# TheCacophonyProject/classifier-pipeline

Measured on AMD Instinct MI355X. Metric: CPTV frames/s end-to-end (track+classify) at 160x120, higher is better.
Workload: dtype u16/i32 track stage (f32 normalise, f64 gates); f32 crop/tile; f32 CNN (stride-1 3x3 convs of stages 2-4 (+ the stride-2 one): two fp16 planes per operand rounded to nearest (11 + 11 significand bits), power-of-two range scaling, 3 fp16 MFMAs per K step, device-side rerun in the exact split if an ac

## Files before the change

### classifier-pipeline_amd/csrc/cpx_api.cpp

```cpp
#include <hip/hip_runtime.h>

#include <algorithm>
#include <cmath>
#include <cstdio>
#include <cstdlib>
#include <cstring>
#include <new>
#include <string>
#include <vector>

#include "cpx_internal.h"
#include "cpx_schedule_core.h"

static_assert(sizeof(cpx_component) == 32, "cpx_component layout is part of the ABI");
static_assert(sizeof(cpx_frame_info) == 80, "cpx_frame_info layout is part of the ABI");
static_assert(sizeof(cpx_frame_meta) == 24, "cpx_frame_meta layout is part of the ABI");
static_assert(sizeof(cpx_config) == 48, "cpx_config layout is part of the ABI");
static_assert(sizeof(cpx_region_ref) == 24 && sizeof(cpx_track_limits) == 32 && sizeof(cpx_crop_req) == 32,
              "classification request layouts are part of the ABI");
static_assert(sizeof(cpx_filter_params) == 72 && sizeof(cpx_track_summary) == 120,
              "end-of-clip layouts are part of the ABI");
static_assert(sizeof(cpx_region) == 56, "cpx_region layout is part of the ABI");
static_assert(sizeof(cpx_track_record) == 32, "cpx_track_record layout is part of the ABI");
static_assert(sizeof(cpx_track_params) == 120, "cpx_track_params layout is part of the ABI");
// ... 79 lines not shown
    return CPX_ERR_HIP;
  }
  h->wtab_len = 65536;
  h->wtab_host.resize(h->wtab_len);
  std::vector<double>& wt = h->wtab_host;
  double w = 0.0;
  for (int k = 0; k < h->wtab_len; ++k) {
    wt[k] = w;
    w = w + cfg->weight_add;
  }
  if (cfg->denoise) {
    if (!cpx::nlm_supported(W, H)) {
      cpx_destroy(h);
      return CPX_ERR_UNSUPPORTED;
    }
    const int fixed_point_mult = (int)(2147483647LL / (21 * 21 * 255));
    std::vector<int> lut(64, 0);
    for (int a2 = 0; a2 < 64; ++a2) {
      const double wv = std::exp(-((double)a2 * (64.0 / 49.0)) / 9.0);
      const double wr = std::nearbyint((double)fixed_point_mult * wv);
      lut[a2] = (wr < 0.001 * fixed_point_mult) ? 0 : (int)wr;
    }
    if (lut[63] != 0 || h->nlm_lut_dev.grow(h, 64 * sizeof(int), "NLM weight table allocation") ||
        hipMemcpy(h->nlm_lut_dev.p, lut.data(), 64 * sizeof(int), hipMemcpyHostToDevice) != hipSuccess) {
      cpx_destroy(h);
      return CPX_ERR_HIP;
    }
  }
  std::vector<uint32_t> thr(h->wtab_len);
  for (int k = 0; k < h->wtab_len; ++k) {
    const double wk = wt[k], m = std::nearbyint(wk);
    const bool exact = (wk == m), near = !exact && std::fabs(wk - m) < 1e-6;
    double hi = near ? m + 1.0 : std::floor(wk) + 1.0;
    if (!(hi >= 0.0)) hi = 0.0;
    if (hi > 536870912.0) hi = 536870912.0;
    thr[k] = 2u * (uint32_t)hi - (near ? 1u : 0u);
  }
  if (h->wthr_dev.grow(h, thr.size() * sizeof(uint32_t), "threshold table allocation") ||
      hipMemcpy(h->wthr_dev.p, thr.data(), thr.size() * sizeof(uint32_t), hipMemcpyHostToDevice) != hipSuccess) {
    cpx_destroy(h);
    return CPX_ERR_HIP;
  }
  if (h->wtab_dev.grow(h, wt.size() * sizeof(double), "weight table allocation") ||
      hipMemcpy(h->wtab_dev.p, wt.data(), wt.size() * sizeof(double), hipMemcpyHostToDevice) != hipSuccess ||
      cpx::frame_kernel_attr_setup() != 0) {
    cpx_destroy(h);
    return CPX_ERR_HIP;
  }
  if (const char* env = std::getenv("CPX_TRACK_PACKED_STATE")) h->packed_state_ok = std::atoi(env) != 0;
  if (const char* env = std::getenv("CPX_CNN_FUSE_CONV1")) h->fuse_conv1 = std::atoi(env) != 0;
  if (const char* env = std::getenv("CPX_TRACK_PER_STEP")) h->track_per_step = std::atoi(env) != 0;
  if (const char* env = std::getenv("CPX_CNN_FUSE_SHORTCUT")) h->fuse_shortcut = std::atoi(env) != 0;
  if (const char* env = std::getenv("CPX_CNN_SHORTCUT_FP16")) h->shortcut_fp16 = std::atoi(env) != 0;
  if (const char* env = std::getenv("CPX_CNN_BLOCK_FUSION")) h->block_fusion = std::min(std::max(std::atoi(env), 0), 2);
  if (const char* env = std::getenv("CPX_CNN_MATH")) {
    if (!std::strcmp(env, "f32")) h->cnn_math = CPX_CNN_MATH_F32;
    else if (!std::strcmp(env, "bf16x3")) h->cnn_math = CPX_CNN_MATH_BF16X3;
    else if (!std::strcmp(env, "bf16x2")) h->cnn_math = CPX_CNN_MATH_BF16X2;
    else if (!std::strcmp(env, "fp16x2")) h->cnn_math = CPX_CNN_MATH_FP16X2;
  }
  *out = h;
  return CPX_OK;
}

static void release_buffers(cpx_handle* h, bool all) {
  for (DeviceBuffer* b : {&h->ws, &h->ws_assoc, &h->bf3_scratch, &h->cnn_arena, &h->graph_arena, &h->ir_scratch}) b->release();
  if (!all) return;
  for (DeviceBuffer* b : {&h->sched, &h->wtab_dev, &h->wthr_dev, &h->nlm_lut_dev, &h->cnn_ovf, &h->ir_bitmap}) b->release();
}

void cpx_destroy(cpx_handle* h) {
  if (!h) return;
  hipSetDevice(h->device);
  if (h->stream) hipStreamSynchronize(h->stream);
  for (cpx_cnn* c : h->cnns) cnn_free(c);
  h->cnns.clear();
  for (cpx_mog2* m : h->mog2s) mog2_free(m);
  h->mog2s.clear();
  for (cpx_graph* g : h->graphs) graph_free(g);
  h->graphs.clear();
  release_buffers(h, true);
  for (auto& e : h->conv_events) {
    hipEventDestroy(e.e0);
    hipEventDestroy(e.e1);
  }
  if (h->stream2) {
    hipStreamSynchronize(h->stream2);
    hipStreamDestroy(h->stream2);
  }
  if (h->ev_median) hipEventDestroy(h->ev_median);
  if (h->ev0) hipEventDestroy(h->ev0);
  if (h->ev1) hipEventDestroy(h->ev1);
  if (h->stream) hipStreamDestroy(h->stream);
  delete h;
}

const char* cpx_last_error(const cpx_handle* h) { return h ? h->err.c_str() : "null handle"; }

void* cpx_stream(cpx_handle* h) { return h ? (void*)h->stream : nullptr; }

static int join_medians(cpx_handle* h) {
  if (h->medians_pending) {
    h->medians_pending = false;
    CPX_HIP(h, hipStreamWaitEvent(h->stream, h->ev_median, 0));
  }
  return CPX_OK;
// ... 711 lines not shown
```

### classifier-pipeline_amd/csrc/cpx_api_cnn.cpp

```cpp
#include <hip/hip_runtime.h>

#include <algorithm>
#include <cmath>
#include <cstdio>
#include <cstdlib>
#include <new>
#include <utility>
#include <vector>

#include "cpx_internal.h"

static_assert(sizeof(cpx_wrresnet_block) == 56 && sizeof(cpx_wrresnet_params) == 1560,
              "cpx_wrresnet_params layout is part of the ABI");

struct cpx_cnn {
  cpx_handle* h = nullptr;
  cpx_wrresnet_params p{};
  std::vector<std::pair<const float*, void*>> split;
  float act_scale[3][CPX_WRRESNET_MAX_BLOCKS][2];
  float res_bound[3] = {0.0f, 0.0f, 0.0f};
  float sc_xscale[3] = {0.0f, 0.0f, 0.0f};
  void* sc_img[3] = {nullptr, nullptr, nullptr};
  double sc_wmax[3] = {-1.0, -1.0, -1.0};
  cpx_cnn() {
// ... 65 lines not shown
    a.sc_H = fuse->H; a.sc_W = fuse->W; a.sc_cin = fuse->cin; a.sc_stride = fuse->stride;
    a.sc_planes = fuse->planes; a.sc_xscale = fuse->xscale;
  }
  return a;
}

class ConvTimer {
 public:
  ConvTimer(cpx_handle* h, bool on) : h_(h) {
    if (!on) return;
    ok_ = hipEventCreate(&ev_.e0) == hipSuccess && hipEventCreate(&ev_.e1) == hipSuccess &&
          hipEventRecord(ev_.e0, h->stream) == hipSuccess;
  }
  ~ConvTimer() {
    if (ev_.e0) hipEventDestroy(ev_.e0);
    if (ev_.e1) hipEventDestroy(ev_.e1);
  }
  ConvTimer(const ConvTimer&) = delete;
  ConvTimer& operator=(const ConvTimer&) = delete;
  bool ok() const { return ok_; }
  int commit(int key, double flops) {
    if (!ev_.e0) return CPX_OK;
    CPX_HIP(h_, hipEventRecord(ev_.e1, h_->stream));
    ev_.key = key;
    ev_.flops = flops;
    h_->conv_events.push_back(ev_);
    ev_ = {};
    return CPX_OK;
  }

 private:
  cpx_handle* h_;
  cpx_handle::ConvEv ev_{};
  bool ok_ = true;
};

enum class ConvRoute {
  Float32,
  Split,
  Fp16Pair,
  RerunOnly,
};

static int conv_run(cpx_handle* h, const cpx_conv_desc* d, const void* split_weights, const conv_fuse* fuse = nullptr,
                    const conv_half* hf = nullptr) {
  if (!h) return CPX_ERR_INVALID;
  if (!d || !d->in_dev || !d->out_dev || !d->weights_dev) return fail(h, CPX_ERR_INVALID, "cpx_conv2d: null argument");
  if (d->N < 1 || d->H < 1 || d->W < 1 || d->groups < 1 || d->Cin % d->groups || d->Cout % d->groups ||
      d->ksize < 1 || d->stride < 1 || (d->in_scale_dev == nullptr) != (d->in_shift_dev == nullptr))
    return fail(h, CPX_ERR_INVALID, "cpx_conv2d: bad descriptor");
  CPX_ENTER(h);
  if (!d->pad_same && (d->H < d->ksize || d->W < d->ksize)) return fail(h, CPX_ERR_INVALID, "cpx_conv2d: input smaller than kernel");
  cpx::ConvArgs a = conv_describe(*d, fuse);
  const bool split = split_math(h) && cpx::conv_bf3_supported(a);
  if (fuse && (!split || a.out_scale || a.residual))
    return fail(h, CPX_ERR_INVALID, "conv_run: shortcut fusion needs the split-operand kernel, no output scale, no residual");
  if (split) a.planes = h->cnn_math == CPX_CNN_MATH_BF16X2 ? 2 : 3;
  const conv_half bare;
  const conv_half& k = hf ? *hf : bare;
  const bool fp16 = split && h->cnn_math == CPX_CNN_MATH_FP16X2;
  const bool aliased = a.out == a.residual || a.out == a.in;
  const bool half = fp16 && cpx::conv_bf3_two_planes(a) && !aliased;
  const bool planes_out = fp16 && k.out_planes;
  const ConvRoute route = k.rerun_only ? ConvRoute::RerunOnly
                          : !split ? ConvRoute::Float32
                          : (half || planes_out) ? ConvRoute::Fp16Pair
                                                 : ConvRoute::Split;
  ConvTimer timer(h, h->conv_timing && route != ConvRoute::RerunOnly);
  if (!timer.ok()) return fail(h, CPX_ERR_HIP, "cpx_conv2d: event creation failed");
  int* word = nullptr;
  if (route == ConvRoute::Fp16Pair || route == ConvRoute::RerunOnly) {
    if (int rc = ensure_ovf_word(h)) return rc;
    if (!k.keep_flag) CPX_HIP(h, hipMemsetAsync(h->cnn_ovf.p, 0, sizeof(int), h->stream));
    word = h->cnn_ovf.as<int>() + k.word;
  }
  if (split && !split_weights) {
    if (int rc = h->bf3_scratch.grow(h, cpx::conv_bf3_weight_bytes(a), "cpx_conv2d: weight scratch allocation failed"))
      return rc;
    cpx::launch_split_weights(a, h->bf3_scratch.p, h->stream);
    split_weights = h->bf3_scratch.p;
  }
  int rc = 0;
  if (route == ConvRoute::Fp16Pair) {
    cpx::ConvArgs first = a;
    if (half) {
      first.planes = 2;
      first.half = 1;
      first.act_scale = k.act_scale;
      first.act_unscale = 1.0f / first.act_scale;
      first.in_planes = k.in_planes;
    }
    first.ovf = word;
    if (planes_out) {
      first.out_planes = 1;
      first.out_act_scale = k.out_act_scale;
    }
    rc = cpx::launch_conv_bf3(first, split_weights, h->stream);
  }
  a.guard = word;
  if (split) {
    if (rc == 0) rc = cpx::launch_conv_bf3(a, split_weights, h->stream);
    if (rc == -3) {
      if (fuse) return fail(h, CPX_ERR_UNSUPPORTED, "conv_run: batch too large for the fused-shortcut kernel (split the call)");
      rc = cpx::launch_conv(a, h->stream);
    }
  } else {
    rc = cpx::launch_conv(a, h->stream);
// ... 573 lines not shown
```

### classifier-pipeline_amd/csrc/cpx_cnn_rw.hip

```cpp
#include <hip/hip_runtime.h>

#include <algorithm>
#include <type_traits>

#include "cpx_kernels.h"

namespace cpx {

namespace {

typedef unsigned u32x4 __attribute__((ext_vector_type(4)));
typedef float f32x4 __attribute__((ext_vector_type(4)));
typedef _Float16 f16x2 __attribute__((ext_vector_type(2)));
typedef _Float16 f16x8 __attribute__((ext_vector_type(8)));

template <typename T>
__device__ __forceinline__ const T* at_off(const T* base, unsigned bytes) {
  return reinterpret_cast<const T*>(reinterpret_cast<const char*>(base) + bytes);
}
template <typename T>
__device__ __forceinline__ T* at_off(T* base, unsigned bytes) {
  return reinterpret_cast<T*>(reinterpret_cast<char*>(base) + bytes);
}
__device__ __forceinline__ unsigned pix_off(int y, int x, int W, int C) {
  return __umul24(__umul24((unsigned)y, (unsigned)W) + (unsigned)x, (unsigned)C);
}
__device__ __forceinline__ float relu_bits(float x) { return __int_as_float(max(__float_as_int(x), 0)); }
__device__ __forceinline__ void split_h(float a, float b, unsigned& hi, unsigned& lo) {
  f16x2 v = {(_Float16)a, (_Float16)b};
  hi = __builtin_bit_cast(unsigned, v);
  asm("v_fma_mixlo_f16 %0, %1, 1.0, -%2 op_sel:[0,0,0] op_sel_hi:[0,0,1]" : "=v"(lo) : "v"(a), "v"(hi));
  asm("v_fma_mixhi_f16 %0, %1, 1.0, -%2 op_sel:[0,0,1] op_sel_hi:[0,0,1]" : "+v"(lo) : "v"(b), "v"(hi));
}
__device__ __forceinline__ f32x4 mfma_h(u32x4 w, u32x4 x, f32x4 c) {
  return __builtin_amdgcn_mfma_f32_16x16x32_f16(__builtin_bit_cast(f16x8, w), __builtin_bit_cast(f16x8, x), c, 0, 0, 0);
}

struct RwTiles {
  unsigned long long m_tx, m_ty;
  int tiles_x, tiles_y, total;
};
template <int I, int N, typename F>
__device__ __forceinline__ void static_for(F&& f) {
  if constexpr (I < N) {
    f(std::integral_constant<int, I>{});
    static_for<I + 1, N>(f);
  }
}
__device__ __forceinline__ int div_magic(int n, unsigned long long m) { return (int)(((unsigned long long)n * m) >> 42); }

constexpr int RW_TW = 16;
constexpr int RW_CT = 256;
constexpr int RW_PPI = RW_CT / 8;
constexpr int RW_WC = 64;

template <int S, int NCH, int ROWS>
struct RwGeo {
  static constexpr int PW = 15 * S + 3, PH = (ROWS - 1) * S + 3, NPX = PH * PW;
  static constexpr int NP = (NPX * 8 + RW_CT - 1) / RW_CT;
  static constexpr int NPXP = (NP * RW_PPI + 3) / 4 * 4 + 2;
  static constexpr int BUF = 2 * 2 * NPXP * 2;
  static constexpr int STEPS = 3 * PH;
  static constexpr int CING = 32 * NCH;
  static constexpr size_t LDS = (size_t)2 * BUF * 16 + (size_t)(2 * CING + 3 * RW_WC) * sizeof(float);
};
constexpr int SC_NPXP = 258;
constexpr int SC_ITEMS = 16 * RW_TW * 8 / RW_CT;
constexpr size_t SC_LDS = (size_t)2 * 2 * SC_NPXP * 2 * 16;

template <int S, int NCH, int ROWS, bool BN, bool RES, bool SC = false>
__global__ __launch_bounds__(RW_CT) __attribute__((amdgpu_waves_per_eu(1, 1))) void conv_rw_kernel(ConvArgs a, const uint4* __restrict__ wimg, RwTiles td) {
  using G = RwGeo<S, NCH, ROWS>;
  constexpr int PW = G::PW, NPX = G::NPX, NP = G::NP, NPXP = G::NPXP, BUF = G::BUF, STEPS = G::STEPS, CING = G::CING, PH = G::PH;
  static_assert(!SC || (S == 1 && NCH == 2 && ROWS == 16 && !RES), "the fp16 shortcut is built into the stride-1 form's two-chunk stream");
  if (*a.ovf != 0) return;
  extern __shared__ __attribute__((aligned(16))) uint4 lds4[];
  uint4* s_buf = lds4;
  float* s_bn = reinterpret_cast<float*>(lds4 + 2 * BUF);
  float* s_par = s_bn + 2 * CING;
  uint4* s_sc = reinterpret_cast<uint4*>(s_par + 3 * RW_WC);
  const int tid = threadIdx.x, lane = tid & 63, wave = tid >> 6, i16 = lane & 15, q = lane >> 4;
  const int ct = wave;
  const int cout_g = a.Cout / a.groups, nhalf = cout_g / RW_WC;
  const int g = blockIdx.y / nhalf, half = blockIdx.y - g * nhalf;
  constexpr bool has_bn = BN;

  u32x4 Wr[NCH][9][2];
  {
    const u32x4* wg = reinterpret_cast<const u32x4*>(wimg) + (size_t)g * NCH * 3 * 24 * cout_g + (q * cout_g + half * RW_WC + ct * 16 + i16);
#pragma unroll
    for (int c = 0; c < NCH; ++c)
#pragma unroll
      for (int ky = 0; ky < 3; ++ky)
#pragma unroll
        for (int kx = 0; kx < 3; ++kx)
#pragma unroll
          for (int p = 0; p < 2; ++p) Wr[c][ky * 3 + kx][p] = wg[(size_t)((c * 3 + ky) * 24 + (p * 3 + kx) * 4) * cout_g];
  }
  u32x4 Wsc[2];
  if constexpr (SC) {
    const u32x4* ws = reinterpret_cast<const u32x4*>(a.sc_planes) + (size_t)g * 8 * cout_g + (q * cout_g + half * RW_WC + ct * 16 + i16);
    Wsc[0] = ws[0];
    Wsc[1] = ws[(size_t)4 * cout_g];
  }
  if (tid < CING) {
    const int ci = g * CING + tid;
    s_bn[tid] = has_bn ? a.in_scale[ci] * a.act_scale : a.act_scale;
    s_bn[CING + tid] = has_bn ? a.in_shift[ci] * a.act_scale : 0.0f;
  }
  if (tid < RW_WC) {
    const int ch = g * cout_g + half * RW_WC + tid;
    float os = a.w_unscale[ch] * a.act_unscale;
    if (a.out_scale) os *= a.out_scale[ch];
    float ob = a.out_shift ? a.out_shift[ch] : 0.0f;
    if (a.sc_in && a.sc_bias) ob += a.sc_bias[ch];
    s_par[tid] = os;
    s_par[RW_WC + tid] = ob;
    s_par[2 * RW_WC + tid] = a.w_scale[ch] * a.act_scale;
  }

  const int per_xcd = (td.total + 7) >> 3;
  auto tile_of = [&](int t) { return (t & 7) * per_xcd + (t >> 3); };
  auto decode = [&](int tile, int& n_, int& oy_, int& ox_) {
    int qd = div_magic(tile, td.m_tx);
    ox_ = (tile - qd * td.tiles_x) * RW_TW;
    tile = qd;
    qd = div_magic(tile, td.m_ty);
// ... 53 lines not shown
    const int iy = oy_ * S - a.pad_top + (ipos[i] >> 8), ix = ox_ * S - a.pad_left + (ipos[i] & 0xFF);
    const bool inside = (unsigned)iy < (unsigned)a.H && (unsigned)ix < (unsigned)a.W;
#pragma unroll
    for (int j = 0; j < 4; ++j) pre_p[i][j] = __float_as_uint(inside ? v[j] : 0.0f);
  };
  auto store_item = [&](const int i, const int bsel) __attribute__((always_inline)) {
    unsigned h0, h1, l0, l1;
    split_h(__uint_as_float(pre_p[i][0]), __uint_as_float(pre_p[i][1]), h0, l0);
    split_h(__uint_as_float(pre_p[i][2]), __uint_as_float(pre_p[i][3]), h1, l1);
    if (has_bn) hmax = pk_max_u16(pk_max_u16(hmax, h0), h1);
    else hmax = pk_max_u16(pk_max_u16(hmax, h0 & 0x7FFF7FFFu), h1 & 0x7FFF7FFFu);
    unsigned char* sp = reinterpret_cast<unsigned char*>(s_buf) + st_base;
    *reinterpret_cast<uint2*>(sp + (bsel * BUF * 16 + i * (RW_PPI * 32))) = make_uint2(h0, h1);
    *reinterpret_cast<uint2*>(sp + (bsel * BUF * 16 + 2 * NPXP * 32 + i * (RW_PPI * 32))) = make_uint2(l0, l1);
  };

  u32x4 pre_s[SC ? SC_ITEMS : 1];
  u32x4 xsh[2], xsl[2];
  const unsigned sc_st_base = (unsigned)((((q8 >> 2) * SC_NPXP + (tid >> 3)) * 4 + (q8 & 3)) * 8);
  const int sc_a_base = ((q >> 1) * SC_NPXP + i16) * 2 + (q & 1);
  auto issue_sc = [&](const int i, const int n_, const int oy_, const int ox_) __attribute__((always_inline)) {
    if constexpr (SC) {
      const float* sc_n = a.sc_in + (size_t)n_ * a.sc_H * a.sc_W * a.sc_cin;
      const int oy = min(oy_ + 2 * i + (tid >> 7), a.Ho - 1), ox = min(ox_ + ((tid >> 3) & 15), a.Wo - 1);
      pre_s[i] = *reinterpret_cast<const u32x4*>(
          at_off(sc_n, (pix_off(oy * a.sc_stride, ox * a.sc_stride, a.sc_W, a.sc_cin) + (unsigned)(g * 32 + 4 * q8)) << 2));
    }
  };
  auto store_sc = [&](const int i) __attribute__((always_inline)) {
    if constexpr (SC) {
      unsigned h0, h1, l0, l1;
      split_h(__uint_as_float(pre_s[i][0]) * a.sc_xscale, __uint_as_float(pre_s[i][1]) * a.sc_xscale, h0, l0);
      split_h(__uint_as_float(pre_s[i][2]) * a.sc_xscale, __uint_as_float(pre_s[i][3]) * a.sc_xscale, h1, l1);
      hmax = pk_max_u16(pk_max_u16(hmax, h0 & 0x7FFF7FFFu), h1 & 0x7FFF7FFFu);
      unsigned char* sp = reinterpret_cast<unsigned char*>(s_sc) + sc_st_base;
      *reinterpret_cast<uint2*>(sp + i * (RW_PPI * 32)) = make_uint2(h0, h1);
      *reinterpret_cast<uint2*>(sp + (2 * SC_NPXP * 32 + i * (RW_PPI * 32))) = make_uint2(l0, l1);
    }
  };

  f32x4 acc[ROWS];
  const int ch_l = g * cout_g + half * RW_WC + ct * 16 + 4 * q;
  auto init_acc = [&]() __attribute__((always_inline)) {
#pragma unroll
    for (int o = 0; o < ROWS; ++o) acc[o] = f32x4{0.0f, 0.0f, 0.0f, 0.0f};
  };
  f32x4 rres[RES ? ROWS : 1];
  auto issue_res = [&](const int o, const int n_, const int oy_, const int ox_) __attribute__((always_inline)) {
    if constexpr (RES) {
      const float* res_n = a.residual + (size_t)n_ * a.Ho * a.Wo * a.Cout;
      const int ox = min(ox_ + i16, a.Wo - 1), oy = min(oy_ + o, a.Ho - 1);
      rres[o] = *reinterpret_cast<const f32x4*>(at_off(res_n, (pix_off(oy, ox, a.Wo, a.Cout) + (unsigned)ch_l) << 2));
    }
  };

  const int a_base = ((q >> 1) * NPXP + S * i16) * 2 + (q & 1);
  constexpr int RW_AHEAD = 3, RW_RING = RW_AHEAD + 1;
  auto compute = [&](auto cc, auto bc, auto&& between) __attribute__((always_inline)) {
    constexpr int C = decltype(cc)::value, B = decltype(bc)::value;
    const uint4* sb = s_buf + B * BUF + a_base;
    u32x4 xh[RW_RING], xl[RW_RING];
    auto frag = [&](auto sc) __attribute__((always_inline)) {
      constexpr int s = decltype(sc)::value;
      constexpr int kx = s / PH, i = s - PH * kx, bf = s % RW_RING;
      xh[bf] = __builtin_bit_cast(u32x4, sb[(i * PW + kx) * 2]);
      xl[bf] = __builtin_bit_cast(u32x4, sb[4 * NPXP + (i * PW + kx) * 2]);
    };
    static_for<0, RW_AHEAD>(frag);
    static_for<0, STEPS>([&](auto sc) __attribute__((always_inline)) {
      constexpr int s = decltype(sc)::value;
      constexpr int kx = s / PH, i = s - PH * kx, bf = s % RW_RING;
      if constexpr (s + RW_AHEAD < STEPS) frag(std::integral_constant<int, s + RW_AHEAD>{});
      static_for<0, 3>([&](auto pc) __attribute__((always_inline)) {
        constexpr int pr = decltype(pc)::value;
        static_for<0, 3>([&](auto rc) __attribute__((always_inline)) {
          constexpr int r = decltype(rc)::value, d = i - r, o = d / S;
          if constexpr (d >= 0 && d % S == 0 && o < ROWS) {
            if constexpr (pr == 0) acc[o] = mfma_h(Wr[C][r * 3 + kx][1], xh[bf], acc[o]);
            if constexpr (pr == 1) acc[o] = mfma_h(Wr[C][r * 3 + kx][0], xl[bf], acc[o]);
            if constexpr (pr == 2) acc[o] = mfma_h(Wr[C][r * 3 + kx][0], xh[bf], acc[o]);
          }
        });
      });
      between(sc);
      __builtin_amdgcn_sched_barrier(0);
    });
  };
  auto unit = [&](auto cc, auto bc, auto ccc, auto cic, auto lastc, const int oyc, const int oxc, const int ni, const int oyi,
                  const int oxi) __attribute__((always_inline)) {
    constexpr int B = decltype(bc)::value, CC = decltype(ccc)::value, CI = decltype(cic)::value;
    constexpr bool LAST = decltype(lastc)::value;
    compute(cc, bc, [&](auto sc) __attribute__((always_inline)) {
      constexpr int s = decltype(sc)::value;
      constexpr int jlo = (s * 3 * NP + STEPS - 1) / STEPS, jhi = ((s + 1) * 3 * NP + STEPS - 1) / STEPS;
      static_for<jlo, (jhi < 3 * NP ? jhi : 3 * NP)>([&](auto jc) __attribute__((always_inline)) {
        constexpr int j = decltype(jc)::value, i = j / 3, k = j % 3;
        if constexpr (k == 0) activate_item(i, CC, oyc, oxc);
        if constexpr (k == 1) store_item(i, B ^ 1);
        if constexpr (k == 2) issue_item(i, CI, ni, oyi, oxi);
      });
      if constexpr (SC && !LAST) {
        constexpr int klo = (s * SC_ITEMS + STEPS - 1) / STEPS, khi = ((s + 1) * SC_ITEMS + STEPS - 1) / STEPS;
        static_for<klo, (khi < SC_ITEMS ? khi : SC_ITEMS)>([&](auto kc) __attribute__((always_inline)) { store_sc(decltype(kc)::value); });
      }
      if constexpr (SC && LAST) {
        if constexpr (s % 3 == 0 && s >= 3 && s / 3 - 1 < ROWS) {
          constexpr int o = s / 3 - 1;
          acc[o] = mfma_h(Wsc[1], xsh[o & 1], acc[o]);
          acc[o] = mfma_h(Wsc[0], xsl[o & 1], acc[o]);
          acc[o] = mfma_h(Wsc[0], xsh[o & 1], acc[o]);
        }
        if constexpr (s % 3 == 0 && s / 3 < ROWS) {
          constexpr int o = s / 3;
          xsh[o & 1] = __builtin_bit_cast(u32x4, s_sc[sc_a_base + o * 2 * RW_TW]);
          xsl[o & 1] = __builtin_bit_cast(u32x4, s_sc[sc_a_base + 4 * SC_NPXP + o * 2 * RW_TW]);
        }
        constexpr int klo = (s * SC_ITEMS + STEPS - 1) / STEPS, khi = ((s + 1) * SC_ITEMS + STEPS - 1) / STEPS;
        static_for<klo, (khi < SC_ITEMS ? khi : SC_ITEMS)>([&](auto kc) __attribute__((always_inline)) { issue_sc(decltype(kc)::value, ni, oyi, oxi); });
      }
      if constexpr (LAST && RES) {
        constexpr int olo = (s * ROWS + STEPS - 1) / STEPS, ohi = ((s + 1) * ROWS + STEPS - 1) / STEPS;
        static_for<olo, (ohi < ROWS ? ohi : ROWS)>([&](auto oc) __attribute__((always_inline)) { issue_res(decltype(oc)::value, n0, oy0, ox0); });
      }
    });
  };

  auto finish = [&](const int n_, const int oy_, const int ox_) __attribute__((always_inline)) {
    const int ox = min(ox_ + i16, a.Wo - 1);
    if (!SC && a.sc_in) {
      const int sc_cg = a.sc_cin / a.groups;
      const float* wsc = a.sc_w + ((size_t)g * sc_cg + q) * cout_g + half * RW_WC + ct * 16 + i16;
      const float ss = s_par[2 * RW_WC + ct * 16 + i16];
      const float* sc_n = a.sc_in + (size_t)n_ * a.sc_H * a.sc_W * a.sc_cin + g * sc_cg + q;
      for (int k4 = 0; k4 < sc_cg; k4 += 4) {
        const float ws = wsc[(size_t)k4 * cout_g] * ss;
#pragma unroll
        for (int o = 0; o < ROWS; ++o) {
          const int oy = min(oy_ + o, a.Ho - 1);
          const float xs = sc_n[((size_t)(oy * a.sc_stride) * a.sc_W + ox * a.sc_stride) * a.sc_cin + k4];
          acc[o] = __builtin_amdgcn_mfma_f32_16x16x4f32(ws, xs, acc[o], 0, 0, 0);
        }
      }
    }
    float* out_n = a.out + (size_t)n_ * a.Ho * a.Wo * a.Cout;
    const f32x4 os = *reinterpret_cast<const f32x4*>(s_par + ct * 16 + 4 * q);
    const f32x4 ob = *reinterpret_cast<const f32x4*>(s_par + RW_WC + ct * 16 + 4 * q);
    const bool xok = ox_ + i16 < a.Wo;
    const unsigned off0 = (pix_off(min(oy_, a.Ho - 1), ox, a.Wo, a.Cout) + (unsigned)ch_l) << 2;
    const unsigned row_bytes = (unsigned)(a.Wo * a.Cout) << 2;
    const bool whole = oy_ + ROWS <= a.Ho;
    auto row = [&](const int o, const bool ok, const unsigned off) __attribute__((always_inline)) {
      f32x4 v;
#pragma unroll
      for (int j = 0; j < 4; ++j) v[j] = __fmaf_rn(acc[o][j], os[j], ob[j]);
      if constexpr (RES) v += rres[o];
      if (a.relu) {
        asm volatile("");
        v.x = relu_bits(v.x); v.y = relu_bits(v.y); v.z = relu_bits(v.z); v.w = relu_bits(v.w);
      }
      if (ok) *reinterpret_cast<f32x4*>(at_off(out_n, off)) = v;
    };
    if (whole) {
#pragma unroll
      for (int o = 0; o < ROWS; ++o) row(o, xok, off0 + (unsigned)o * row_bytes);
    } else {
#pragma unroll
      for (int o = 0; o < ROWS; ++o) row(o, xok && oy_ + o < a.Ho, off0 + (unsigned)min(o, a.Ho - 1 - oy_) * row_bytes);
    }
  };

#pragma unroll
  for (int i = 0; i < NP; ++i) issue_item(i, 0, n0, oy0, ox0);
  __syncthreads();
#pragma unroll
  for (int c = 0; c < NCH; ++c) {
    psc[c] = *reinterpret_cast<const f32x4*>(s_bn + c * 32 + 4 * q8);
    psh[c] = *reinterpret_cast<const f32x4*>(s_bn + CING + c * 32 + 4 * q8);
  }
#pragma unroll
  for (int i = 0; i < NP; ++i) {
    activate_item(i, 0, oy0, ox0);
    store_item(i, 0);
  }
  using I0 = std::integral_constant<int, 0>;
  using I1 = std::integral_constant<int, 1>;
  using Yes = std::integral_constant<bool, true>;
  using No = std::integral_constant<bool, false>;
  if constexpr (NCH == 2) {
#pragma unroll
    for (int i = 0; i < NP; ++i) issue_item(i, 1, n0, oy0, ox0);
    if constexpr (SC) {
#pragma unroll
      for (int i = 0; i < SC_ITEMS; ++i) issue_sc(i, n0, oy0, ox0);
    }
    init_acc();
    for (;;) {
      n1 = n0; oy1 = oy0; ox1 = ox0;
      const bool more = advance(n1, oy1, ox1);
      __syncthreads();
      unit(I0{}, I0{}, I1{}, I0{}, No{}, oy0, ox0, n1, oy1, ox1);
      __syncthreads();
      unit(I1{}, I1{}, I0{}, I1{}, Yes{}, oy1, ox1, n1, oy1, ox1);
// ... 32 lines not shown

__global__ __launch_bounds__(256) void split_shortcut_kernel(const float* __restrict__ w, uint4* __restrict__ out, int groups, int cin_g,
                                                             int cout_g, const float* __restrict__ wscale, float factor) {
  const int nch = cin_g / 32;
  const int total = groups * nch * 4 * cout_g;
  const int idx = blockIdx.x * blockDim.x + threadIdx.x;
  if (idx >= total) return;
  const int col = idx % cout_g;
  int r = idx / cout_g;
  const int qq = r & 3;
  r >>= 2;
  const int chunk = r % nch, g = r / nch;
  const float f = wscale[g * cout_g + col] * factor;
  float v[8];
#pragma unroll
  for (int j = 0; j < 8; ++j) v[j] = w[((size_t)g * cin_g + chunk * 32 + 8 * qq + j) * cout_g + col] * f;
  uint4 hi, lo;
  split_h(v[0], v[1], hi.x, lo.x);
  split_h(v[2], v[3], hi.y, lo.y);
  split_h(v[4], v[5], hi.z, lo.z);
  split_h(v[6], v[7], hi.w, lo.w);
  const size_t base = (size_t)(g * nch + chunk) * 8 * cout_g + (size_t)qq * cout_g + col;
  out[base] = hi;
  out[base + (size_t)4 * cout_g] = lo;
}

}

bool conv_shortcut_planes_layer(const ConvArgs& second, int sc_cin_g) {
  if (conv_rw_kind(second) == 1) return sc_cin_g == 32;
  return second.ksize == 3 && second.stride == 1 && second.groups >= 1 && second.Cin == second.Cout &&
         second.Cout == 128 * second.groups && sc_cin_g == 64;
}
size_t conv_shortcut_image_bytes(int groups, int cin_g, int cout_g) { return (size_t)groups * (cin_g / 32) * 8 * cout_g * 16; }
void launch_split_shortcut(const float* sc_w, void* img, int groups, int cin_g, int cout_g, const float* w_scale, float factor,
                           hipStream_t s) {
  const int total = groups * (cin_g / 32) * 4 * cout_g;
  hipLaunchKernelGGL(split_shortcut_kernel, dim3((unsigned)((total + 255) / 256)), dim3(256), 0, s, sc_w, reinterpret_cast<uint4*>(img),
                     groups, cin_g, cout_g, w_scale, factor);
}

int conv_rw_kind(const ConvArgs& a) {
  if (a.ksize != 3 || a.groups < 1 || a.Cin % a.groups || a.Cout % a.groups) return 0;
  const int cin_g = a.Cin / a.groups, cout_g = a.Cout / a.groups;
  int kind = 0;
  if (a.stride == 1 && cin_g == 64 && cout_g == 64) kind = 1;
  else if (a.stride == 2 && cin_g == 32 && cout_g == 64) kind = 2;
  else if (a.stride == 3 && cin_g == 64 && cout_g == 128) kind = 3;
  return kind;
}
bool conv_rw_layer(const ConvArgs& a) { return conv_rw_kind(a) == 1; }

namespace {
template <int S, int NCH, int ROWS, bool BN, bool RES, bool SC = false>
int launch_rw_t(const ConvArgs& a, const uint4* wimg, hipStream_t s) {
  using G = RwGeo<S, NCH, ROWS>;
  constexpr size_t LDS = G::LDS + (SC ? SC_LDS : 0);
  static_assert(LDS <= 160 * 1024 - 1024, "two chunk buffers (and the shortcut's operand) must fit the CU's LDS");
  RwTiles td{};
  td.tiles_x = (a.Wo + RW_TW - 1) / RW_TW;
  td.tiles_y = (a.Ho + ROWS - 1) / ROWS;
  const long long tiles = (long long)td.tiles_x * td.tiles_y * a.N;
  if (tiles >= (1 << 22) - 8 || td.tiles_x >= 4096 || td.tiles_y >= 4096) return -3;
  td.m_tx = (1ull << 42) / td.tiles_x + 1;
  td.m_ty = (1ull << 42) / td.tiles_y + 1;
  td.total = (int)tiles;
  static bool lds_ready[64];
  if (!cpx_dyn_lds_ready(reinterpret_cast<const void*>(conv_rw_kernel<S, NCH, ROWS, BN, RES, SC>), lds_ready, 160 * 1024 - 1024)) return -1;
  static int cus_of[64];
  int dev = 0;
  if (hipGetDevice(&dev) != hipSuccess || dev < 0 || dev >= 64) return -1;
  if (cus_of[dev] == 0) {
    int cus = 256;
    if (hipDeviceGetAttribute(&cus, hipDeviceAttributeMultiprocessorCount, dev) != hipSuccess || cus < 8) cus = 256;
    cus_of[dev] = cus;
  }
  const int ny = a.groups * ((a.Cout / a.groups) / RW_WC);
  int gx = std::max(8, cus_of[dev] / ny / 8 * 8);
  gx = (int)std::min<long long>(gx, (tiles + 7) / 8 * 8);
  hipLaunchKernelGGL((conv_rw_kernel<S, NCH, ROWS, BN, RES, SC>), dim3((unsigned)gx, (unsigned)ny), dim3(RW_CT), LDS, s, a, wimg, td);
  return 0;
}
}

int launch_conv_rw(const ConvArgs& a, const void* wimg, hipStream_t s) {
  const int kind = conv_rw_kind(a);
  if (!kind || !a.half || a.planes != 2 || a.ovf == nullptr || a.in_planes || a.out_planes) return -2;
  if ((long long)a.H * a.W >= (1 << 24) || (long long)a.Ho * a.Wo >= (1 << 24)) return -3;
  if (a.sc_in && ((a.sc_cin / a.groups) & 3)) return -2;
  const uint4* wi = reinterpret_cast<const uint4*>(wimg);
  const bool bn = a.in_scale != nullptr, res = a.residual != nullptr;
  if (kind == 1) {
    if (a.pad_top != 1 || a.pad_left != 1 || a.H != a.Ho || a.W != a.Wo) return -2;
    if (a.sc_in && a.sc_planes) {
      if (bn || res || !conv_shortcut_planes_layer(a, a.sc_cin / a.groups) || a.sc_stride < 1 || !(a.sc_xscale > 0.0f) ||
          (a.sc_H - 1) / a.sc_stride + 1 != a.Ho || (a.sc_W - 1) / a.sc_stride + 1 != a.Wo)
        return -2;
      if ((long long)a.sc_H * a.sc_W >= (1 << 24) || (long long)a.sc_H * a.sc_W * a.sc_cin >= (1ll << 30)) return -3;
      return launch_rw_t<1, 2, 16, false, false, true>(a, wi, s);
    }
    if (bn && res) return launch_rw_t<1, 2, 16, true, true>(a, wi, s);
    if (bn) return launch_rw_t<1, 2, 16, true, false>(a, wi, s);
    if (res) return launch_rw_t<1, 2, 16, false, true>(a, wi, s);
    return launch_rw_t<1, 2, 16, false, false>(a, wi, s);
  }
  if (res || a.sc_in || a.pad_top < 0 || a.pad_top > 1 || a.pad_left < 0 || a.pad_left > 1) return -2;
  if (kind == 2) return bn ? launch_rw_t<2, 1, 8, true, false>(a, wi, s) : launch_rw_t<2, 1, 8, false, false>(a, wi, s);
  return bn ? launch_rw_t<3, 2, 4, true, false>(a, wi, s) : launch_rw_t<3, 2, 4, false, false>(a, wi, s);
}

}
```

### classifier-pipeline_amd/csrc/cpx_internal.h

```cpp
#pragma once
#include <hip/hip_runtime.h>

#include <map>
#include <string>
#include <vector>

#include "cpx.h"
#include "cpx_kernels.h"

struct cpx_cnn;
struct cpx_mog2;
struct cpx_graph;
void cnn_free(cpx_cnn* c);
void graph_free(cpx_graph* g);
void mog2_free(cpx_mog2* m);

struct DeviceBuffer {
  void* p = nullptr;
  size_t bytes = 0;
  DeviceBuffer() = default;
  DeviceBuffer(const DeviceBuffer&) = delete;
  DeviceBuffer& operator=(const DeviceBuffer&) = delete;
  int grow(cpx_handle* h, size_t need, const char* what);
  void release() {
    if (p) hipFree(p);
    p = nullptr;
    bytes = 0;
  }
  template <class T>
  T* as() const { return static_cast<T*>(p); }
};

struct cpx_handle {
  int device = 0;
  cpx_config cfg{};
  hipStream_t stream = nullptr;
  std::string err;
  DeviceBuffer ws;
  DeviceBuffer wtab_dev, wthr_dev;
  int wtab_len = 0;
  std::vector<double> wtab_host;
  DeviceBuffer nlm_lut_dev;
  DeviceBuffer sched;
  struct ConvEv { int key; double flops; hipEvent_t e0, e1; };
  std::vector<ConvEv> conv_events;
  bool conv_timing = false;
  DeviceBuffer ws_assoc;
  hipEvent_t ev0 = nullptr, ev1 = nullptr;
  int last_launches = 0;
  bool timing_valid = false;
  hipStream_t stream2 = nullptr;
  bool state_packed = false;
  bool packed_state_ok = true;
  bool fuse_conv1 = true;
  bool medians_pending = false;
  hipEvent_t ev_median = nullptr;
  bool track_per_step = false;
  std::vector<struct cpx_cnn*> cnns;
  std::vector<struct cpx_mog2*> mog2s;
  std::vector<struct cpx_graph*> graphs;
  DeviceBuffer graph_arena;
  int stream_frames = -1;
  int stream_assoc_frames = -1;
  bool stream_filt_state = false;
  int last_B = 0;
  struct StagedBackground { std::vector<uint16_t> bg, kcnt; double average; };
  std::map<int, StagedBackground> staged_bg;
  int cnn_math = CPX_CNN_MATH_FP16X2;
  bool fuse_shortcut = true;
  bool shortcut_fp16 = true;
  DeviceBuffer bf3_scratch;
  DeviceBuffer cnn_arena;
  DeviceBuffer cnn_ovf;
  int block_fusion = 2;
  DeviceBuffer ir_scratch;
  DeviceBuffer ir_bitmap;
};

inline int fail(cpx_handle* h, int code, const char* what, hipError_t e = hipSuccess) {
  if (h) {
    h->err = what;
    if (e != hipSuccess) {
      h->err += ": ";
      h->err += hipGetErrorString(e);
    }
  }
  return code;
}

#define CPX_HIP(h, call)                                            \
  do {                                                              \
    hipError_t _e = (call);                                         \
    if (_e != hipSuccess) return fail((h), CPX_ERR_HIP, #call, _e); \
  } while (0)

#define CPX_ENTER(h)                           \
  do {                                         \
    CPX_HIP((h), hipSetDevice((h)->device));   \
    (void)hipGetLastError();                   \
  } while (0)

inline int DeviceBuffer::grow(cpx_handle* h, size_t need, const char* what) {
  if (need <= bytes) return CPX_OK;
  if (p) CPX_HIP(h, hipStreamSynchronize(h->stream));
  release();
  const hipError_t e = hipMalloc(&p, need);
  if (e != hipSuccess) {
    p = nullptr;
    (void)hipGetLastError();
    return fail(h, CPX_ERR_NOMEM, what, e);
  }
  bytes = need;
  return CPX_OK;
}

inline size_t align_up(size_t v, size_t a) { return (v + a - 1) / a * a; }
```

### classifier-pipeline_amd/csrc/cpx_kernels.h

```cpp
#pragma once
#include <hip/hip_runtime.h>
#include <stddef.h>
#include <stdint.h>

#include "cpx.h"

#ifndef CPX_TRACK_THREADS
#define CPX_TRACK_THREADS 768
#endif
#ifndef CPX_TRACK_CHUNKS
#define CPX_TRACK_CHUNKS 7
#endif
#ifndef CPX_TRACK_LDS_COMPONENTS
#define CPX_TRACK_LDS_COMPONENTS 256
#endif
#ifndef CPX_TRACK_MIN_WAVES_PER_SIMD
#define CPX_TRACK_MIN_WAVES_PER_SIMD 6
#endif

namespace cpx {

typedef cpx_component Component;
typedef cpx_frame_info FrameInfo;

// ... 113 lines not shown
  int W, H, crop_x, crop_y, crop_w, crop_h;
  int frame_size, square_width;
  int limits_flags;
  const uint16_t* frames;
  const float* filtered;
  const FrameInfo* info;
  const cpx_region_ref* refs;
  const int* track_offsets;
  cpx_track_limits* limits;
  const cpx_crop_req* reqs;
  float* out;
};
struct AggregateArgs {
  int n_samples, n_tracks, n_labels, fp_index, square_width;
  const float* probs;
  const int* sample_track;
  const cpx_crop_req* reqs;
  float* scores;
  int* best;
};
void launch_aggregate(const AggregateArgs& a, hipStream_t s);
void launch_limits(const ClassifyArgs& a, int n_tracks, hipStream_t s);
void launch_crop(const ClassifyArgs& a, int n_reqs, hipStream_t s);

struct ConvArgs {
  int N, H, W, Cin, Cout, groups, ksize, stride, relu;
  int Ho, Wo, pad_top, pad_left;
  const float* in;
  float* out;
  const float* weights;
  const float* in_scale;
  const float* in_shift;
  const float* out_scale;
  const float* out_shift;
  const float* residual;
  const float* sc_in;
  const float* sc_w;
  const float* sc_bias;
  int sc_H, sc_W, sc_cin, sc_stride;
  const void* sc_planes;
  float sc_xscale;
  const float* c1_in;
  const float* c1_w;
  const float* c1_b;
  int planes;
  int half;
  float act_scale, act_unscale;
  const float* w_scale;
  const float* w_unscale;
  int* ovf;
  const int* guard;
  int out_planes, in_planes;
  float out_act_scale;
};
struct HeadArgs {
  int N, HW, C, L;
  int n_hidden, activation;
  int hidden_sizes[CPX_HEAD_MAX_HIDDEN];
  const float* in;
  const float* bn_scale;
  const float* bn_shift;
  const float* hidden_w[CPX_HEAD_MAX_HIDDEN];
  const float* hidden_b[CPX_HEAD_MAX_HIDDEN];
  const float* dense_w;
  const float* dense_b;
  float* logits;
  float* probs;
};
int launch_conv(const ConvArgs& a, hipStream_t s);
bool conv_bf3_supported(const ConvArgs& a);
size_t conv_bf3_weight_bytes(const ConvArgs& a);
bool conv_bf3_two_planes(const ConvArgs& a);
bool conv_bf3_can_store_planes(const ConvArgs& a);
bool conv_bf3_can_load_planes(const ConvArgs& a);
void launch_split_weights(const ConvArgs& a, void* wimg, hipStream_t s);
int launch_conv_bf3(const ConvArgs& a, const void* wimg, hipStream_t s);
bool conv_block32_supported(const ConvArgs& a, const ConvArgs& b);
int launch_conv_block32(const ConvArgs& a, const ConvArgs& b, const void* wimg_a, const void* wimg_b, hipStream_t s);
int launch_conv_block32s(const ConvArgs& a, const ConvArgs& b, const void* wa, const void* wb, hipStream_t s);
int conv_rw_kind(const ConvArgs& a);
bool conv_rw_layer(const ConvArgs& a);
int launch_conv_rw(const ConvArgs& a, const void* wimg, hipStream_t s);
bool conv_shortcut_planes_layer(const ConvArgs& second, int sc_cin_g);
size_t conv_shortcut_image_bytes(int groups, int cin_g, int cout_g);
void launch_split_shortcut(const float* sc_w, void* img, int groups, int cin_g, int cout_g, const float* w_scale, float factor,
                           hipStream_t s);
const float* conv_bf3_weight_scales(const ConvArgs& a, const void* wimg);
void launch_head(const HeadArgs& a, hipStream_t s);
void launch_count_overflow(int* ovf, int n_words, hipStream_t s);

struct CptvArgs {
  int W, H;
  const unsigned char* payload;
  const long long* frame_offsets;
  const int* bit_widths;
  const int* clip_offsets;
  uint16_t* frames_out;
};
int launch_cptv_unpack(const CptvArgs& a, int B, hipStream_t s);

struct CptvInflateArgs {
  int B;
  const unsigned char* in;
  const cpx_cptv_file* files;
  unsigned char* out;
  cpx_cptv_frame_slot* slots;
// ... 140 lines not shown
```

Measured before the change: 3.161 million.

## Stream conv output rows during the last channel chunk instead of after it

Adds a RIDE variant of the row-window conv kernel. During the last input-channel chunk it applies BN scale/bias, residual and ReLU to each output row as soon as that row's final tap product is done, and stores it with a buffer store. Residual loads are respread to arrive before they are needed, and the activation item schedule is compressed. The aim is to hide the epilogue's stores and residual reads behind the remaining MFMA stream. It is enabled by default behind CPX_CNN_RW_RIDE, and adds scheduling barriers and register pressure that may disturb the pipeline.

New measurement: 3.180 million (median of 6 runs). Within noise of the previous version (+0.6%).

```diff
diff --git a/classifier-pipeline_amd/csrc/cpx_api.cpp b/classifier-pipeline_amd/csrc/cpx_api.cpp
--- a/classifier-pipeline_amd/csrc/cpx_api.cpp
+++ b/classifier-pipeline_amd/csrc/cpx_api.cpp
@@ -155,6 +155,7 @@
   if (const char* env = std::getenv("CPX_TRACK_PER_STEP")) h->track_per_step = std::atoi(env) != 0;
   if (const char* env = std::getenv("CPX_CNN_FUSE_SHORTCUT")) h->fuse_shortcut = std::atoi(env) != 0;
   if (const char* env = std::getenv("CPX_CNN_SHORTCUT_FP16")) h->shortcut_fp16 = std::atoi(env) != 0;
+  if (const char* env = std::getenv("CPX_CNN_RW_RIDE")) h->rw_ride = std::atoi(env) != 0;
   if (const char* env = std::getenv("CPX_CNN_BLOCK_FUSION")) h->block_fusion = std::min(std::max(std::atoi(env), 0), 2);
   if (const char* env = std::getenv("CPX_CNN_MATH")) {
     if (!std::strcmp(env, "f32")) h->cnn_math = CPX_CNN_MATH_F32;
diff --git a/classifier-pipeline_amd/csrc/cpx_api_cnn.cpp b/classifier-pipeline_amd/csrc/cpx_api_cnn.cpp
--- a/classifier-pipeline_amd/csrc/cpx_api_cnn.cpp
+++ b/classifier-pipeline_amd/csrc/cpx_api_cnn.cpp
@@ -141,7 +141,8 @@
   CPX_ENTER(h);
   if (!d->pad_same && (d->H < d->ksize || d->W < d->ksize)) return fail(h, CPX_ERR_INVALID, "cpx_conv2d: input smaller than kernel");
   cpx::ConvArgs a = conv_describe(*d, fuse);
-  const bool split = split_math(h) && cpx::conv_bf3_supported(a);
+  a.rw_ride = h->rw_ride;
+  const bool split =split_math(h) && cpx::conv_bf3_supported(a);
   if (fuse && (!split || a.out_scale || a.residual))
     return fail(h, CPX_ERR_INVALID, "conv_run: shortcut fusion needs the split-operand kernel, no output scale, no residual");
   if (split) a.planes = h->cnn_math == CPX_CNN_MATH_BF16X2 ? 2 : 3;
diff --git a/classifier-pipeline_amd/csrc/cpx_cnn_rw.hip b/classifier-pipeline_amd/csrc/cpx_cnn_rw.hip
--- a/classifier-pipeline_amd/csrc/cpx_cnn_rw.hip
+++ b/classifier-pipeline_amd/csrc/cpx_cnn_rw.hip
@@ -68,11 +68,15 @@
 constexpr int SC_ITEMS = 16 * RW_TW * 8 / RW_CT;
 constexpr size_t SC_LDS = (size_t)2 * 2 * SC_NPXP * 2 * 16;
 
-template <int S, int NCH, int ROWS, bool BN, bool RES, bool SC = false>
+template <int S, int NCH, int ROWS, bool BN, bool RES, bool SC = false, bool RIDE = false>
 __global__ __launch_bounds__(RW_CT) __attribute__((amdgpu_waves_per_eu(1, 1))) void conv_rw_kernel(ConvArgs a, const uint4* __restrict__ wimg, RwTiles td) {
   using G = RwGeo<S, NCH, ROWS>;
   constexpr int PW = G::PW, NPX = G::NPX, NP = G::NP, NPXP = G::NPXP, BUF = G::BUF, STEPS = G::STEPS, CING = G::CING, PH = G::PH;
   static_assert(!SC || (S == 1 && NCH == 2 && ROWS == 16 && !RES), "the fp16 shortcut is built into the stride-1 form's two-chunk stream");
+  constexpr int RIDE0 = 2 * PH + 3;
+  static_assert(!RIDE || S < 3, "measured at stride 1 and 2 only");
+  static_assert(RIDE0 + S * (ROWS - 1) >= STEPS, "row ROWS - 1 is complete with the last step: its epilogue stays behind the stream");
+  static_assert(!SC || 3 * (ROWS - 1) + 3 < 2 * PH + 2 + (ROWS - 1), "a row's shortcut products (step 3 o + 3) lie before its last tap product (step 2 PH + 2 + o)");
   if (*a.ovf != 0) return;
   extern __shared__ __attribute__((aligned(16))) uint4 lds4[];
   uint4* s_buf = lds4;
@@ -232,6 +236,29 @@
       const int ox = min(ox_ + i16, a.Wo - 1), oy = min(oy_ + o, a.Ho - 1);
       rres[o] = *reinterpret_cast<const f32x4*>(at_off(res_n, (pix_off(oy, ox, a.Wo, a.Cout) + (unsigned)ch_l) << 2));
     }
+  };
+  f32x4 eos, eob;
+  unsigned eoff = 0u;
+  __amdgpu_buffer_rsrc_t orsrc;
+  const int relu_floor = a.relu ? 0 : (int)0x80000000;
+  const unsigned row_bytes = (unsigned)(a.Wo * a.Cout) << 2;
+  auto ride_begin = [&](const int n_, const int oy_, const int ox_) __attribute__((always_inline)) {
+    float* out_n = a.out + (size_t)n_ * a.Ho * a.Wo * a.Cout;
+    orsrc = __builtin_amdgcn_make_buffer_rsrc(out_n, 0, (int)(a.Ho * row_bytes), 0x00020000);
+    const unsigned off0 = (pix_off(oy_, min(ox_ + i16, a.Wo - 1), a.Wo, a.Cout) + (unsigned)ch_l) << 2;
+    eoff = ox_ + i16 < a.Wo ? off0 : 0x80000000u;
+    eos = *reinterpret_cast<const f32x4*>(s_par + ct * 16 + 4 * q);
+    eob = *reinterpret_cast<const f32x4*>(s_par + RW_WC + ct * 16 + 4 * q);
+  };
+  auto ride_row = [&](const int o, const int oy_) __attribute__((always_inline)) {
+    f32x4 v;
+#pragma unroll
+    for (int j = 0; j < 4; ++j) v[j] = __fmaf_rn(acc[o][j], eos[j], eob[j]);
+    if constexpr (RES) v += rres[o];
+#pragma unroll
+    for (int j = 0; j < 4; ++j) v[j] = __int_as_float(max(__float_as_int(v[j]), relu_floor));
+    const unsigned roff = oy_ + o < a.Ho ? (unsigned)o * row_bytes : 0x40000000u;
+    __builtin_amdgcn_raw_buffer_store_b128(__builtin_bit_cast(u32x4, v), orsrc, (int)(eoff + roff), 0, 0);
   };
 
   const int a_base = ((q >> 1) * NPXP + S * i16) * 2 + (q & 1);
@@ -253,6 +280,7 @@
       if constexpr (s + RW_AHEAD < STEPS) frag(std::integral_constant<int, s + RW_AHEAD>{});
       static_for<0, 3>([&](auto pc) __attribute__((always_inline)) {
         constexpr int pr = decltype(pc)::value;
+        if constexpr (RIDE && C == NCH - 1 && pr == 1 && s >= RIDE0 && (s - RIDE0) % S == 0) __builtin_amdgcn_sched_barrier(0);
         static_for<0, 3>([&](auto rc) __attribute__((always_inline)) {
           constexpr int r = decltype(rc)::value, d = i - r, o = d / S;
           if constexpr (d >= 0 && d % S == 0 && o < ROWS) {
@@ -272,7 +300,8 @@
     constexpr bool LAST = decltype(lastc)::value;
     compute(cc, bc, [&](auto sc) __attribute__((always_inline)) {
       constexpr int s = decltype(sc)::value;
-      constexpr int jlo = (s * 3 * NP + STEPS - 1) / STEPS, jhi = ((s + 1) * 3 * NP + STEPS - 1) / STEPS;
+      constexpr int DS = RIDE && LAST ? RIDE0 : STEPS;
+      constexpr int jlo = (s * 3 * NP + DS - 1) / DS, jhi = ((s + 1) * 3 * NP + DS - 1) / DS;
       static_for<jlo, (jhi < 3 * NP ? jhi : 3 * NP)>([&](auto jc) __attribute__((always_inline)) {
         constexpr int j = decltype(jc)::value, i = j / 3, k = j % 3;
         if constexpr (k == 0) activate_item(i, CC, oyc, oxc);
@@ -298,14 +327,28 @@
         constexpr int klo = (s * SC_ITEMS + STEPS - 1) / STEPS, khi = ((s + 1) * SC_ITEMS + STEPS - 1) / STEPS;
         static_for<klo, (khi < SC_ITEMS ? khi : SC_ITEMS)>([&](auto kc) __attribute__((always_inline)) { issue_sc(decltype(kc)::value, ni, oyi, oxi); });
       }
-      if constexpr (LAST && RES) {
+      if constexpr (LAST && RES && RIDE) {
+        static_assert(2 * S * (ROWS - 1) + PH <= RIDE0 + S * (ROWS - 1), "a kx pass between a row's request and its use");
+        if constexpr (s % (2 * S) == 0 && s / (2 * S) < ROWS) issue_res(s / (2 * S), n0, oy0, ox0);
+      }
+      if constexpr (LAST && RES && !RIDE) {
         constexpr int olo = (s * ROWS + STEPS - 1) / STEPS, ohi = ((s + 1) * ROWS + STEPS - 1) / STEPS;
         static_for<olo, (ohi < ROWS ? ohi : ROWS)>([&](auto oc) __attribute__((always_inline)) { issue_res(decltype(oc)::value, n0, oy0, ox0); });
       }
+      if constexpr (LAST && RIDE) {
+        if constexpr (s == 0) ride_begin(n0, oy0, ox0);
+        if constexpr (s >= RIDE0 && (s - RIDE0) % S == 0) ride_row((s - RIDE0) / S, oy0);
+      }
     });
   };
 
   auto finish = [&](const int n_, const int oy_, const int ox_) __attribute__((always_inline)) {
+    if constexpr (RIDE) {
+      static_for<0, ROWS>([&](auto oc) __attribute__((always_inline)) {
+        if constexpr (RIDE0 + S * decltype(oc)::value >= STEPS) ride_row(decltype(oc)::value, oy_);
+      });
+      return;
+    }
     const int ox = min(ox_ + i16, a.Wo - 1);
     if (!SC && a.sc_in) {
       const int sc_cg = a.sc_cin / a.groups;
@@ -327,7 +370,6 @@
     const f32x4 ob = *reinterpret_cast<const f32x4*>(s_par + RW_WC + ct * 16 + 4 * q);
     const bool xok = ox_ + i16 < a.Wo;
     const unsigned off0 = (pix_off(min(oy_, a.Ho - 1), ox, a.Wo, a.Cout) + (unsigned)ch_l) << 2;
-    const unsigned row_bytes = (unsigned)(a.Wo * a.Cout) << 2;
     const bool whole = oy_ + ROWS <= a.Ho;
     auto row = [&](const int o, const bool ok, const unsigned off) __attribute__((always_inline)) {
       f32x4 v;
@@ -466,7 +508,7 @@
 bool conv_rw_layer(const ConvArgs& a) { return conv_rw_kind(a) == 1; }
 
 namespace {
-template <int S, int NCH, int ROWS, bool BN, bool RES, bool SC = false>
+template <int S, int NCH, int ROWS, bool BN, bool RES, bool SC = false, bool RIDE = false>
 int launch_rw_t(const ConvArgs& a, const uint4* wimg, hipStream_t s) {
   using G = RwGeo<S, NCH, ROWS>;
   constexpr size_t LDS = G::LDS + (SC ? SC_LDS : 0);
@@ -480,7 +522,7 @@
   td.m_ty = (1ull << 42) / td.tiles_y + 1;
   td.total = (int)tiles;
   static bool lds_ready[64];
-  if (!cpx_dyn_lds_ready(reinterpret_cast<const void*>(conv_rw_kernel<S, NCH, ROWS, BN, RES, SC>), lds_ready, 160 * 1024 - 1024)) return -1;
+  if (!cpx_dyn_lds_ready(reinterpret_cast<const void*>(conv_rw_kernel<S, NCH, ROWS, BN, RES, SC, RIDE>), lds_ready, 160 * 1024 - 1024)) return -1;
   static int cus_of[64];
   int dev = 0;
   if (hipGetDevice(&dev) != hipSuccess || dev < 0 || dev >= 64) return -1;
@@ -492,8 +534,12 @@
   const int ny = a.groups * ((a.Cout / a.groups) / RW_WC);
   int gx = std::max(8, cus_of[dev] / ny / 8 * 8);
   gx = (int)std::min<long long>(gx, (tiles + 7) / 8 * 8);
-  hipLaunchKernelGGL((conv_rw_kernel<S, NCH, ROWS, BN, RES, SC>), dim3((unsigned)gx, (unsigned)ny), dim3(RW_CT), LDS, s, a, wimg, td);
+  hipLaunchKernelGGL((conv_rw_kernel<S, NCH, ROWS, BN, RES, SC, RIDE>), dim3((unsigned)gx, (unsigned)ny), dim3(RW_CT), LDS, s, a, wimg, td);
   return 0;
+}
+template <int S, int NCH, int ROWS, bool BN, bool RES, bool SC = false>
+int launch_rw_r(bool ride, const ConvArgs& a, const uint4* wimg, hipStream_t s) {
+  return ride ? launch_rw_t<S, NCH, ROWS, BN, RES, SC, true>(a, wimg, s) : launch_rw_t<S, NCH, ROWS, BN, RES, SC, false>(a, wimg, s);
 }
 }
 
@@ -504,6 +550,7 @@
   if (a.sc_in && ((a.sc_cin / a.groups) & 3)) return -2;
   const uint4* wi = reinterpret_cast<const uint4*>(wimg);
   const bool bn = a.in_scale != nullptr, res = a.residual != nullptr;
+  const bool ride = a.rw_ride && (long long)a.Ho * a.Wo * a.Cout * 4 <= (1ll << 30) && !(a.sc_in && !a.sc_planes);
   if (kind == 1) {
     if (a.pad_top != 1 || a.pad_left != 1 || a.H != a.Ho || a.W != a.Wo) return -2;
     if (a.sc_in && a.sc_planes) {
@@ -511,15 +558,15 @@
           (a.sc_H - 1) / a.sc_stride + 1 != a.Ho || (a.sc_W - 1) / a.sc_stride + 1 != a.Wo)
         return -2;
       if ((long long)a.sc_H * a.sc_W >= (1 << 24) || (long long)a.sc_H * a.sc_W * a.sc_cin >= (1ll << 30)) return -3;
-      return launch_rw_t<1, 2, 16, false, false, true>(a, wi, s);
-    }
-    if (bn && res) return launch_rw_t<1, 2, 16, true, true>(a, wi, s);
-    if (bn) return launch_rw_t<1, 2, 16, true, false>(a, wi, s);
-    if (res) return launch_rw_t<1, 2, 16, false, true>(a, wi, s);
-    return launch_rw_t<1, 2, 16, false, false>(a, wi, s);
+      return launch_rw_r<1, 2, 16, false, false, true>(ride, a, wi, s);
+    }
+    if (bn && res) return launch_rw_r<1, 2, 16, true, true>(ride, a, wi, s);
+    if (bn) return launch_rw_r<1, 2, 16, true, false>(ride, a, wi, s);
+    if (res) return launch_rw_r<1, 2, 16, false, true>(ride, a, wi, s);
+    return launch_rw_r<1, 2, 16, false, false>(ride, a, wi, s);
   }
   if (res || a.sc_in || a.pad_top < 0 || a.pad_top > 1 || a.pad_left < 0 || a.pad_left > 1) return -2;
-  if (kind == 2) return bn ? launch_rw_t<2, 1, 8, true, false>(a, wi, s) : launch_rw_t<2, 1, 8, false, false>(a, wi, s);
+  if (kind == 2) return bn ? launch_rw_r<2, 1, 8, true, false>(ride, a, wi, s) : launch_rw_r<2, 1, 8, false, false>(ride, a, wi, s);
   return bn ? launch_rw_t<3, 2, 4, true, false>(a, wi, s) : launch_rw_t<3, 2, 4, false, false>(a, wi, s);
 }
 
diff --git a/classifier-pipeline_amd/csrc/cpx_internal.h b/classifier-pipeline_amd/csrc/cpx_internal.h
--- a/classifier-pipeline_amd/csrc/cpx_internal.h
+++ b/classifier-pipeline_amd/csrc/cpx_internal.h
@@ -69,6 +69,7 @@
   int cnn_math = CPX_CNN_MATH_FP16X2;
   bool fuse_shortcut = true;
   bool shortcut_fp16 = true;
+  bool rw_ride = true;
   DeviceBuffer bf3_scratch;
   DeviceBuffer cnn_arena;
   DeviceBuffer cnn_ovf;
diff --git a/classifier-pipeline_amd/csrc/cpx_kernels.h b/classifier-pipeline_amd/csrc/cpx_kernels.h
--- a/classifier-pipeline_amd/csrc/cpx_kernels.h
+++ b/classifier-pipeline_amd/csrc/cpx_kernels.h
@@ -189,6 +189,7 @@
   const int* guard;
   int out_planes, in_planes;
   float out_act_scale;
+  int rw_ride;
 };
 struct HeadArgs {
   int N, HW, C, L;
```
